# sacs-epfl/decentralized-learning-simulator

Measured on AMD Instinct MI355X. Metric: device-resident GB/s, N-way weighted model-tensor reduce; 1/2/4/8 MI355X, higher is better.
Workload: dtype f32

## Files before the change

decentralized-learning-simulator_amd/csrc/dispatch.hpp:

```cpp
#pragma once

#include <hip/hip_runtime.h>

#include <algorithm>
#include <cmath>
#include <cstdint>
#include <cstdlib>
#include <cstring>
#include <type_traits>
#include <vector>

#include "dlsim.h"
#include "wreduce_kernels.hpp"
#include "chunk_mean_kernels.hpp"
#include "ab_env.hpp"


namespace dlsim_host __attribute__((visibility("hidden"))) {

int fail(int code, const char* fmt, ...) __attribute__((format(printf, 2, 3)));
int hip_fail(hipError_t e, const char* what);

constexpr int kVpt = 4;
constexpr size_t kBatchSmallBytes = size_t{1} << 20;
// ... 446 lines not shown
    fi.push_back(fan_in[t]);
    dv.push_back(divs ? divs[t] : 1.0f);
  }
  const int g = static_cast<int>(group.size());
  const size_t tile1 = dlsim::kBlock;
  int t0 = 0;
  while (t0 < g) {
    int t1 = t0, ptrs = 0;
    uint64_t blocks = 0;
    while (t1 < g && t1 - t0 < dlsim::kBatchMaxTasks && ptrs + fi[t1] <= dlsim::kBatchMaxPtrs &&
           blocks + ne[t1] / Op::E / tile1 + 1 < 0x7fffffffull) {
      ptrs += fi[t1];
      blocks += ne[t1] / Op::E / tile1 + 1;
      ++t1;
    }
    hipError_t e = launch_batch<Op>(fi.data(), ioff.data(), ins.data(), ws.data(), dv.data(), os.data(),
                                    ne.data(), t0, t1, st);
    if (e != hipSuccess) return hip_fail(e, "batched kernel launch");
    t0 = t1;
  }
  return DLSIM_OK;
}

struct TableLayout {
  size_t tasks_off, map_off, ptrs_off, w_off, bytes;
  uint32_t nblocks;
  int vpt;
};

inline size_t round8(size_t x) { return (x + 7) / 8 * 8; }

template <class Op>
uint32_t task_blocks(size_t nelem, int vpt) {
  const size_t tile = static_cast<size_t>(dlsim::kBlock) * vpt;
  return static_cast<uint32_t>(nelem / Op::E / tile + 1);
}

template <class Op>
bool table_layout(int b, const int* fan_in, const size_t* nelem, TableLayout* L) {
  uint64_t blocks = 0, ptrs = 0;
  L->vpt = batch_vpt<Op>(nelem, 0, b);
  for (int t = 0; t < b; ++t) {
    blocks += task_blocks<Op>(nelem[t], L->vpt);
    ptrs += static_cast<uint64_t>(fan_in[t]);
  }
  if (blocks >= 0x7fffffffull) return false;
  L->nblocks = static_cast<uint32_t>(blocks);
  L->tasks_off = round8(sizeof(dlsim::BatchTableHeader));
  L->map_off = round8(L->tasks_off + sizeof(dlsim::BatchTaskDesc) * static_cast<size_t>(b));
  L->ptrs_off = round8(L->map_off + sizeof(uint32_t) * static_cast<size_t>(blocks));
  L->w_off = round8(L->ptrs_off + sizeof(void*) * static_cast<size_t>(ptrs));
  L->bytes = round8(L->w_off + sizeof(float) * static_cast<size_t>(ptrs));
  return true;
}

template <class Op>
int table_fill(int b, const int* fan_in, const void* const* in, const float* w, void* const* outs,
               const size_t* nelem, void* h_table, size_t bytes) {
  TableLayout L;
  if (!table_layout<Op>(b, fan_in, nelem, &L)) return fail(DLSIM_E_ARG, "batch too large");
  if (bytes < L.bytes) return fail(DLSIM_E_ARG, "table buffer too small (%zu < %zu)", bytes, L.bytes);
  if (cross_task_overlap(b, fan_in, in, outs, nelem, Op::kBytes))
    return fail(DLSIM_E_ARG,
                "a task's output overlaps another task's input or output: one table launch runs all tasks "
                "concurrently (use separate calls, or dlsim_wreduce_batched, which orders them)");
  unsigned char* base = static_cast<unsigned char*>(h_table);
  std::memset(base, 0, L.bytes);
  auto* h = reinterpret_cast<dlsim::BatchTableHeader*>(base);
  auto* tasks = reinterpret_cast<dlsim::BatchTaskDesc*>(base + L.tasks_off);
  auto* map = reinterpret_cast<uint32_t*>(base + L.map_off);
  auto* ptrs = reinterpret_cast<const void**>(base + L.ptrs_off);
  auto* ws = reinterpret_cast<float*>(base + L.w_off);
  h->ntasks = static_cast<uint32_t>(b);
  h->nblocks = L.nblocks;
  h->vpt = static_cast<uint32_t>(L.vpt);
  h->tasks_off = L.tasks_off;
  h->map_off = L.map_off;
  h->ptrs_off = L.ptrs_off;
  h->w_off = L.w_off;
  uint32_t blk = static_cast<uint32_t>(b), off = 0;
  bool uniform = true;
  for (int t = 0; t < b; ++t) {
    const size_t total = nelem[t] * Op::kBytes;
    if (fan_in[t] > DLSIM_MAX_FUSED_INPUTS || total > kMaxLaunchOutBytes || !aligned16(outs[t]))
      return fail(DLSIM_E_ARG, "task %d cannot be table-batched (fan-in <= %d, 16-B aligned, < 2 GiB)", t,
                  DLSIM_MAX_FUSED_INPUTS);
    const uint32_t nb = task_blocks<Op>(nelem[t], L.vpt);
    tasks[t].out = outs[t];
    tasks[t].nvec = nelem[t] / Op::E;
    tasks[t].nelem = nelem[t];
    tasks[t].block_start = blk - 1;
    tasks[t].ptr_off = off;
    tasks[t].fan_in = static_cast<uint32_t>(fan_in[t]);
    map[t] = static_cast<uint32_t>(t);
    for (uint32_t k = 0; k + 1 < nb; ++k) map[blk + k] = static_cast<uint32_t>(t);
    for (int i = 0; i < fan_in[t]; ++i) {
      if (!aligned16(in[off + i]))
        return fail(DLSIM_E_ARG, "task %d input %d is not 16-byte aligned", t, i);
      ptrs[off + i] = in[off + i];
      ws[off + i] = w[off + i];
    }
    blk += nb - 1;
    off += static_cast<uint32_t>(fan_in[t]);
    uniform = uniform && fan_in[t] == fan_in[0];
  }
  h->uniform_fan_in = uniform ? static_cast<uint32_t>(fan_in[0]) : 0u;
  return DLSIM_OK;
}

template <class Op, int NF, int VPT>
hipError_t launch_table_nf(const void* d_table, uint32_t blocks, hipStream_t st) {
  hipLaunchKernelGGL((dlsim::k_wreduce_batch_table<Op, NF, group_size<Op>(), VPT, kNT, store_policy<Op>(),
                                                    kBatchWave<Op, VPT>>),
                     dim3(blocks), dim3(dlsim::kBlock), 0, st, static_cast<const unsigned char*>(d_table));
  return hipGetLastError();
}

template <class Op, int K, int VPT>
hipError_t launch_table_fixed(const void* d_table, int n, uint32_t blocks, hipStream_t st) {
  if constexpr (K > max_fixed_fan_in<Op>()) {
    return launch_table_nf<Op, 0, VPT>(d_table, blocks, st);
  } else {
    if (n == K) return launch_table_nf<Op, K, VPT>(d_table, blocks, st);
    return launch_table_fixed<Op, K + 1, VPT>(d_table, n, blocks, st);
  }
}

template <class Op>
int table_launch(const void* h_table, const void* d_table, hipStream_t st) {
  const auto* h = static_cast<const dlsim::BatchTableHeader*>(h_table);
  if (h->ntasks == 0) return DLSIM_OK;
  if (h->vpt != 1 && h->vpt != 4)
    return fail(DLSIM_E_ARG, "not a table written by dlsim_batch_table_fill (vectors per lane %u)", h->vpt);
  const int n = static_cast<int>(h->uniform_fan_in);
  hipError_t e;
  if (h->vpt == 1)
    e = n ? launch_table_fixed<Op, 1, 1>(d_table, n, h->nblocks, st) : launch_table_nf<Op, 0, 1>(d_table, h->nblocks, st);
  else
    e = n ? launch_table_fixed<Op, 1, 4>(d_table, n, h->nblocks, st) : launch_table_nf<Op, 0, 4>(d_table, h->nblocks, st);
  if (e != hipSuccess) return hip_fail(e, "table batch launch");
  return DLSIM_OK;
}


inline size_t chunk_mean_ilp_begin(int m, size_t n, int threads, size_t esz = 4, size_t vw = 8) {
  if (n <= 1) return 0;
  const size_t rnd = 128 / esz;
  size_t b = 0, e = n;
  if (!(static_cast<unsigned long long>(m) * n < 32768ULL || threads <= 1)) {
    const size_t tp = static_cast<size_t>(threads) < n ? static_cast<size_t>(threads) : n;
    const size_t cs = (n + tp - 1) / tp;
    for (size_t t = 0; t < tp; ++t) {
      size_t tb = t * cs;
      if (tb >= n) break;
      size_t te = tb + cs < n ? tb + cs : n;
      tb -= tb % rnd;
      if (te != n) te -= te % rnd;
      if (tb < te) {
        b = tb;
        e = te;
      }
    }
  }
// ... 278 lines not shown
      continue;
    }
    if (static_cast<int>(batch.size()) == dlsim::kCmMaxTasks || np + m > dlsim::kCmMaxPtrs ||
        tiles + tb > 0x7fffffffu) {
      int rc = flush();
      if (rc != DLSIM_OK) return rc;
    }
    batch.push_back({t, ib, flags, head});
    np += m;
    tiles += tb;
  }
  return flush();
}

}

#define DLSIM_REDUCE_ENTRIES(X, Op)                                                                      \
  X int dlsim_host::run<Op>(const void* const*, int, const float*, void*, size_t, hipStream_t, float);  \
  X int dlsim_host::run_batched<Op>(int, const int*, const void* const*, const float*, void* const*,    \
                                    const size_t*, hipStream_t, const float*);                          \
  X bool dlsim_host::table_layout<Op>(int, const int*, const size_t*, dlsim_host::TableLayout*);        \
  X int dlsim_host::table_fill<Op>(int, const int*, const void* const*, const float*, void* const*,     \
                                   const size_t*, void*, size_t);                                       \
  X int dlsim_host::table_launch<Op>(const void*, const void*, hipStream_t);
#define DLSIM_MEAN_ENTRIES(X, Op)                                                                        \
  X int dlsim_host::run<Op>(const void* const*, int, const float*, void*, size_t, hipStream_t, float);  \
  X int dlsim_host::run_batched<Op>(int, const int*, const void* const*, const float*, void* const*,    \
                                    const size_t*, hipStream_t, const float*);                          \
  X int dlsim_host::run_chunk_mean<Op>(int, const int*, const void* const*, void* const*, const size_t*, \
                                       int, hipStream_t, std::vector<dlsim_host::ChunkMeanPlan>*, int);
#define DLSIM_PROBE_ENTRIES(X, Op) \
  X int dlsim_host::run<Op>(const void* const*, int, const float*, void*, size_t, hipStream_t, float);
#define DLSIM_F64_ENTRIES(X, Op) \
  X int dlsim_host::run<Op>(const void* const*, int, const double*, void*, size_t, hipStream_t, float);
#define DLSIM_CHUNK_ENTRIES(X, Op)                                                                       \
  X int dlsim_host::run_chunk_mean<Op>(int, const int*, const void* const*, void* const*, const size_t*, \
                                       int, hipStream_t, std::vector<dlsim_host::ChunkMeanPlan>*, int);

#define DLSIM_ALL_ENTRIES(X)                  \
  DLSIM_REDUCE_ENTRIES(X, dlsim::F32Exact)    \
  DLSIM_REDUCE_ENTRIES(X, dlsim::F32Fast)     \
  DLSIM_REDUCE_ENTRIES(X, dlsim::BF16Exact)   \
  DLSIM_REDUCE_ENTRIES(X, dlsim::BF16Fast)    \
  DLSIM_REDUCE_ENTRIES(X, dlsim::F16Exact)    \
  DLSIM_REDUCE_ENTRIES(X, dlsim::F16Fast)     \
  DLSIM_MEAN_ENTRIES(X, dlsim::F32Mean)       \
  DLSIM_MEAN_ENTRIES(X, dlsim::BF16Mean)      \
// ... 7 lines not shown
```

decentralized-learning-simulator_amd/csrc/dlsim_abi.hip:

```cpp
#include <hip/hip_runtime.h>

#include <algorithm>
#include <cstdarg>
#include <cstdio>
#include <cstdint>
#include <cstdlib>
#include <cstring>
#include <mutex>
#include <string>
#include <thread>
#include <vector>

#include "abi_common.hpp"
#include "dispatch.hpp"
#include "fanin_checks.hpp"

#include "host_pack.hpp"

namespace dlsim_host __attribute__((visibility("hidden"))) {

template <class F>
int with_policy(int dtype, int mode, F&& f) {
  const bool fast = mode == DLSIM_FAST;
  if (dtype == DLSIM_F32) return fast ? f(dlsim::F32Fast{}) : f(dlsim::F32Exact{});
// ... 393 lines not shown
                           size_t table_bytes) {
  g_err.clear();
  if (b < 0 || !h_table) return fail(DLSIM_E_ARG, "bad arguments");
  if (b > 0 && (!fan_in || !d_inputs || !h_weights || !d_outs || !n_elems))
    return fail(DLSIM_E_ARG, "null array argument");
  size_t off = 0;
  for (int t = 0; t < b; ++t) {
    int rc = check_args(d_inputs + off, fan_in[t], h_weights + off, d_outs[t], n_elems[t], dtype, DLSIM_EXACT);
    if (rc != DLSIM_OK) return fail(rc, "task %d: %s", t, g_err.c_str());
    off += static_cast<size_t>(fan_in[t]);
  }
  return with_policy(dtype, DLSIM_EXACT, [&](auto op) {
    return table_fill<decltype(op)>(b, fan_in, d_inputs, h_weights, d_outs, n_elems, h_table, table_bytes);
  });
}

int dlsim_batch_table_launch(const void* h_table, const void* d_table, int dtype, int mode, void* stream) {
  g_err.clear();
  if (!h_table || !d_table) return fail(DLSIM_E_ARG, "null table");
  if (!known_dtype(dtype)) return dtype_fail(dtype);
  if (mode != DLSIM_EXACT && mode != DLSIM_FAST) return fail(DLSIM_E_MODE, "unsupported mode %d", mode);
  hipStream_t st = static_cast<hipStream_t>(stream);
  return with_policy(dtype, mode, [&](auto op) { return table_launch<decltype(op)>(h_table, d_table, st); });
}

int dlsim_mean(const void* const* d_inputs, int n, void* d_out, size_t n_elems, int dtype,
               void* stream) {
  g_err.clear();
  int rc = check_args(d_inputs, n, nullptr, d_out, n_elems, dtype, DLSIM_EXACT, false);
  if (rc != DLSIM_OK) return rc;
  hipStream_t st = static_cast<hipStream_t>(stream);
  const float div = static_cast<float>(n);
  return with_mean_policy(dtype, [&](auto op) {
    return run<decltype(op)>(d_inputs, n, nullptr, d_out, n_elems, st, div);
  });
}

int dlsim_mean_batched(int b, const int* fan_in, const void* const* d_inputs, void* const* d_outs,
                       const size_t* n_elems, int dtype, void* stream) {
  g_err.clear();
  if (b < 0) return fail(DLSIM_E_ARG, "b must be >= 0 (got %d)", b);
  if (b == 0) return DLSIM_OK;
  if (!fan_in || !d_inputs || !d_outs || !n_elems) return fail(DLSIM_E_ARG, "null array argument");
  size_t off = 0;
  std::vector<float> divs(static_cast<size_t>(b));
  for (int t = 0; t < b; ++t) {
// ... 1054 lines not shown
```

decentralized-learning-simulator_amd/csrc/wreduce_kernels.hpp:

```cpp
#pragma once

#include <hip/hip_runtime.h>
#include <stdint.h>

#include <type_traits>

#pragma clang fp contract(off)

namespace dlsim {

constexpr int kBlock = 256;

typedef uint32_t u32x4 __attribute__((ext_vector_type(4)));
typedef float f32x2 __attribute__((ext_vector_type(2)));
typedef __bf16 bf16x2 __attribute__((ext_vector_type(2)));

__device__ __forceinline__ float bf16_round(float f) {
  uint32_t u = __float_as_uint(f);
  if ((u & 0x7fffffffu) > 0x7f800000u) return __uint_as_float(0x7fc00000u);
  u += 0x7fffu + ((u >> 16) & 1u);
  return __uint_as_float(u & 0xffff0000u);
}

__device__ __forceinline__ void bf16_round2(float& a0, float& a1) {
// ... 754 lines not shown
    if (full * kTile < nvec)
      reduce_tile<Op, TaskArgs, NF, G, VPT, NT, true, STP>(a, n, o, full * kTile + threadIdx.x, nvec);
    const size_t j = nvec * Op::E + threadIdx.x;
    if (j < s.nelem[t]) fold_scalar<Op, TaskArgs>(a, n, s.out[t], j);
    return;
  }
  if constexpr (WAVEMAP) {
    const size_t lane_off = (threadIdx.x >> 6) * 64 * VPT + (threadIdx.x & 63);
    reduce_tile<Op, TaskArgs, NF, G, VPT, NT, false, STP, 64>(a, n, o, (local - 1) * kTile + lane_off, nvec);
  } else {
    reduce_tile<Op, TaskArgs, NF, G, VPT, NT, false, STP>(a, n, o, (local - 1) * kTile + threadIdx.x, nvec);
  }
}

struct BatchTableHeader {
  uint32_t ntasks;
  uint32_t nblocks;
  uint32_t uniform_fan_in;
  uint32_t vpt;
  uint64_t tasks_off;
  uint64_t map_off;
  uint64_t ptrs_off;
  uint64_t w_off;
};

struct BatchTaskDesc {
  void* out;
  uint64_t nvec;
  uint64_t nelem;
  uint32_t block_start;
  uint32_t ptr_off;
  uint32_t fan_in;
  uint32_t reserved;
};

struct TableArgs {
  const void* const* p;
  const float* w;
  __device__ const void* ptr(int i) const { return p[i]; }
  __device__ float wt(int i) const { return w[i]; }
  __device__ float divisor() const { return 1.0f; }
};

template <class Op, int NF, int G, int VPT, int NT, int STP, bool WAVEMAP = false>
__global__ __launch_bounds__(kBlock) void k_wreduce_batch_table(const unsigned char* __restrict__ table) {
  const BatchTableHeader* h = reinterpret_cast<const BatchTableHeader*>(table);
  const uint32_t* map = reinterpret_cast<const uint32_t*>(table + h->map_off);
// ... 2 lines not shown
  const TableArgs a{reinterpret_cast<const void* const*>(table + h->ptrs_off) + d.ptr_off,
                    reinterpret_cast<const float*>(table + h->w_off) + d.ptr_off};
  const int n = NF > 0 ? NF : static_cast<int>(d.fan_in);
  const size_t nvec = d.nvec;
  constexpr size_t kTile = static_cast<size_t>(kBlock) * VPT;
  const size_t full = nvec / kTile;
  const OutRef o = make_out<STP>(d.out, nvec);
  const uint32_t local = blockIdx.x < h->ntasks ? 0u : blockIdx.x - d.block_start;
  if (local == 0) {
    if (full * kTile < nvec)
      reduce_tile<Op, TableArgs, NF, G, VPT, NT, true, STP>(a, n, o, full * kTile + threadIdx.x, nvec);
    const size_t j = nvec * Op::E + threadIdx.x;
    if (j < d.nelem) fold_scalar<Op, TableArgs>(a, n, d.out, j);
    return;
  }
  if constexpr (WAVEMAP) {
    const size_t lane_off = (threadIdx.x >> 6) * 64 * VPT + (threadIdx.x & 63);
    reduce_tile<Op, TableArgs, NF, G, VPT, NT, false, STP, 64>(a, n, o, (local - 1) * kTile + lane_off, nvec);
  } else {
    reduce_tile<Op, TableArgs, NF, G, VPT, NT, false, STP>(a, n, o, (local - 1) * kTile + threadIdx.x, nvec);
  }
}

template <int BYTES>
struct XorProbe {
  static constexpr int E = 16 / BYTES;
  static constexpr int kBytes = BYTES;
  static constexpr int kFmt = BYTES == 4 ? kFmtF32 : kFmtBF16;
  __device__ static float init(float) { return 0.0f; }
  __device__ static float step(float acc, float, float x) {
    float r = __uint_as_float(__float_as_uint(acc) ^ __float_as_uint(x));
    asm volatile("" : "+v"(r));
    return r;
  }
  __device__ static void step2(float& a0, float& a1, float w, float x0, float x1) {
    a0 = step(a0, w, x0);
    a1 = step(a1, w, x1);
  }
  __device__ static float finish(float a, float) { return a; }
};

constexpr int kMixedMaxInputs = 32;
struct MixedSlots {
  const void* p[kMixedMaxInputs];
  double w[kMixedMaxInputs];
  int dt[kMixedMaxInputs];
// ... 68 lines not shown
```

decentralized-learning-simulator_amd/dasklearn_amd/_native.py:

```python
from __future__ import annotations

import ctypes
import os
import threading
from typing import Optional, Sequence

import numpy as np

LIB_DIR = os.path.join(os.path.dirname(os.path.abspath(__file__)), "lib")
LIB_PATH = os.path.join(LIB_DIR, "libdlsim_hip.so")

DLSIM_F32 = 0
DLSIM_BF16 = 1
DLSIM_F16 = 2
DLSIM_F64 = 3
DLSIM_EXACT = 0
DLSIM_FAST = 1
MAX_FUSED_INPUTS = 128
DLSIM_E_ARG = -1
DLSIM_E_RCCL = -4
DLSIM_E_PEER = -5
DLSIM_E_DISAGREE = -6
DLSIM_GATHER_NONE = 0
DLSIM_GATHER_BCAST = 1
DLSIM_GATHER_ALLGATHER = 2


def ab_env(name: str, default: Optional[str] = None) -> Optional[str]:
    if os.environ.get("DLSIM_AB") != "1":
        return default
    return os.environ.get(name, default)

EXPORTS = (
    "dlsim_wreduce",
    "dlsim_wreduce_f64",
    "dlsim_wreduce_tensors",
    "dlsim_wreduce_batched",
    "dlsim_batch_table_bytes",
    "dlsim_batch_table_fill",
    "dlsim_batch_table_launch",
    "dlsim_mean",
    "dlsim_mean_batched",
    "dlsim_chunk_mean_batched",
    "dlsim_chunk_mean_ilp_begin",
    "dlsim_chunk_mean_plan",
    "dlsim_rccl_bind",
    "dlsim_wreduce_sharded",
    "dlsim_wreduce_sharded_f64",
    "dlsim_wreduce_mixed",
    "dlsim_sgd_step",
    "dlsim_sgd_step_tensors",
    "dlsim_sgd_momentum_step",
    "dlsim_sgd_momentum_step_tensors",
    "dlsim_robust_reduce",
    "dlsim_robust_reduce_tensors",
    "dlsim_robust_reduce_batched",
    "dlsim_robust_batch_geometry",
    "dlsim_robust_reduce_tensors_batched",
    "dlsim_robust_nearest_reduce",
    "dlsim_robust_nearest_reduce_tensors",
    "dlsim_pairwise_sqdist",
    "dlsim_pairwise_sqdist_tensors",
    "dlsim_pairdist_geometry",
# ... 14 lines not shown
    "dlsim_sharded_plan_run_f64",
    "dlsim_sharded_plan_destroy",
    "dlsim_host_wreduce",
    "dlsim_host_wreduce_zc",
    "dlsim_host_wreduce_resident",
    "dlsim_host_chunk_mean",
    "dlsim_host_pack",
    "dlsim_shard_range",
    "dlsim_probe_pattern",
    "dlsim_kernel_name",
    "dlsim_last_error",
    "dlsim_version",
)

_lib = None
_lock = threading.Lock()


class ChunkLaunch(ctypes.Structure):
    _fields_ = [("form", ctypes.c_int), ("mf", ctypes.c_int), ("rows", ctypes.c_int), ("bpt", ctypes.c_int),
                ("grid", ctypes.c_uint), ("ntasks", ctypes.c_int), ("first_task", ctypes.c_int)]


CHUNK_FORMS = ("tiled_few", "tiled", "table", "defer_rf4", "defer_rf8", "defer_m")


class DlsimError(RuntimeError):

    def __init__(self, fn: str, rc: int, msg: str):
        super().__init__(f"{fn} failed (rc={rc}): {msg}")
        self.rc = rc


def load() -> ctypes.CDLL:
    global _lib
    if _lib is not None:
        return _lib
    with _lock:
        if _lib is not None:
            return _lib
        if not os.path.exists(LIB_PATH):
            raise ImportError(
                f"HIP extension not built: {LIB_PATH} is missing. Run "
                "`python -c 'import __graft_entry__ as g; g.build()'` at the repo root.")
        lib = ctypes.CDLL(LIB_PATH)
        vp, sz, i = ctypes.c_void_p, ctypes.c_size_t, ctypes.c_int
        lib.dlsim_wreduce.argtypes = [ctypes.POINTER(vp), i, ctypes.POINTER(ctypes.c_float), vp,
                                      sz, i, i, vp]
        lib.dlsim_wreduce.restype = i
        lib.dlsim_wreduce_f64.argtypes = [ctypes.POINTER(vp), i, ctypes.POINTER(ctypes.c_double), vp, sz, i, vp]
        lib.dlsim_wreduce_f64.restype = i
        lib.dlsim_wreduce_tensors.argtypes = [ctypes.POINTER(vp), i, i, ctypes.POINTER(sz),
                                              ctypes.POINTER(ctypes.c_float), ctypes.POINTER(vp),
                                              i, i, vp]
        lib.dlsim_wreduce_tensors.restype = i
        lib.dlsim_wreduce_batched.argtypes = [i, ctypes.POINTER(i), ctypes.POINTER(vp),
                                              ctypes.POINTER(ctypes.c_float), ctypes.POINTER(vp),
                                              ctypes.POINTER(sz), i, i, vp]
        lib.dlsim_wreduce_batched.restype = i
        lib.dlsim_batch_table_bytes.argtypes = [i, ctypes.POINTER(i), ctypes.POINTER(sz), i,
                                                ctypes.POINTER(sz)]
        lib.dlsim_batch_table_bytes.restype = i
        lib.dlsim_batch_table_fill.argtypes = [i, ctypes.POINTER(i), ctypes.POINTER(vp),
                                               ctypes.POINTER(ctypes.c_float), ctypes.POINTER(vp),
                                               ctypes.POINTER(sz), i, vp, sz]
        lib.dlsim_batch_table_fill.restype = i
        lib.dlsim_batch_table_launch.argtypes = [vp, vp, i, i, vp]
        lib.dlsim_batch_table_launch.restype = i
        lib.dlsim_mean.argtypes = [ctypes.POINTER(vp), i, vp, sz, i, vp]
        lib.dlsim_mean.restype = i
        lib.dlsim_mean_batched.argtypes = [i, ctypes.POINTER(i), ctypes.POINTER(vp), ctypes.POINTER(vp),
                                           ctypes.POINTER(sz), i, vp]
        lib.dlsim_mean_batched.restype = i
        lib.dlsim_chunk_mean_batched.argtypes = [i, ctypes.POINTER(i), ctypes.POINTER(vp), ctypes.POINTER(vp),
                                                 ctypes.POINTER(sz), i, i, vp]
        lib.dlsim_chunk_mean_batched.restype = i
        lib.dlsim_chunk_mean_ilp_begin.argtypes = [i, sz, i]
        lib.dlsim_chunk_mean_ilp_begin.restype = sz
        lib.dlsim_chunk_mean_plan.argtypes = [i, ctypes.POINTER(i), ctypes.POINTER(vp), ctypes.POINTER(vp),
                                              ctypes.POINTER(sz), i, i, i, ctypes.POINTER(ChunkLaunch), i,
                                              ctypes.POINTER(i)]
        lib.dlsim_chunk_mean_plan.restype = i
        lib.dlsim_rccl_bind.argtypes = [ctypes.c_char_p]
        lib.dlsim_rccl_bind.restype = i
        lib.dlsim_wreduce_sharded.argtypes = [ctypes.POINTER(vp), sz, i, ctypes.POINTER(ctypes.c_float), vp, sz, i,
                                              i, vp, i, vp]
        lib.dlsim_wreduce_sharded.restype = i
        lib.dlsim_wreduce_sharded_f64.argtypes = [ctypes.POINTER(vp), sz, i, ctypes.POINTER(ctypes.c_double), vp,
                                                  sz, i, vp, i, vp]
        lib.dlsim_wreduce_sharded_f64.restype = i
        lib.dlsim_sharded_plan_create.argtypes = [vp, sz, i, i, i, vp, ctypes.POINTER(vp)]
# ... 688 lines not shown
            numels.append(out.numel())
        lib = load()
        c_fan = (ctypes.c_int * self.b)(*fan)
        c_num = (ctypes.c_size_t * self.b)(*numels)
        nbytes = ctypes.c_size_t(0)
        _check("dlsim_batch_table_bytes",
               lib.dlsim_batch_table_bytes(self.b, c_fan, c_num, self.dtype, ctypes.byref(nbytes)))
        self._h = torch.empty(nbytes.value, dtype=torch.uint8, pin_memory=True)
        _check("dlsim_batch_table_fill",
               lib.dlsim_batch_table_fill(self.b, c_fan, (ctypes.c_void_p * len(ptrs))(*ptrs),
                                          (ctypes.c_float * len(ws))(*ws),
                                          (ctypes.c_void_p * self.b)(*outs), c_num, self.dtype,
                                          self._h.data_ptr(), nbytes.value))
        self._d = self._h.to(self.device, non_blocking=True)
        torch.cuda.current_stream(self.device).synchronize()
        self._keep = tasks
        self._lib = lib

    def launch(self, stream=None) -> None:
        _check("dlsim_batch_table_launch",
               self._lib.dlsim_batch_table_launch(self._h.data_ptr(), self._d.data_ptr(), self.dtype,
                                                  self.mode, _stream_handle(self.device, stream)))


def wreduce_batched(tasks, mode: int = DLSIM_EXACT, stream=None):
    lib = load()
    b = len(tasks)
    if b == 0:
        return []
    dt = dtype_code(tasks[0][2].dtype)
    fan, ptrs, ws, outs, numels = [], [], [], [], []
    for inputs, w32, out in tasks:
        if len(inputs) < 1:
            raise IndexError("list index out of range")
        if len(w32) != len(inputs):
            raise AssertionError("weights/models length mismatch")
        for t in list(inputs) + [out]:
            if not t.is_cuda or t.dtype != out.dtype or t.numel() != out.numel() or not t.is_contiguous() \
                    or t.device != out.device:
                raise ValueError("each task: contiguous device tensors of one dtype, size and device")
        if out.dtype != tasks[0][2].dtype or out.device != tasks[0][2].device:
            raise ValueError("all tasks of a batch share dtype and device")
        fan.append(len(inputs))
        ptrs.extend(t.data_ptr() for t in inputs)
        ws.extend(np.asarray(w32, dtype=np.float32).tolist())
        outs.append(out.data_ptr())
# ... 549 lines not shown
```

include/dlsim.h:

```cpp
#ifndef DLSIM_H_
#define DLSIM_H_

#include <stddef.h>
#include <stdint.h>

#ifdef __cplusplus
extern "C" {
#endif

enum dlsim_dtype {
  DLSIM_F32 = 0,
  DLSIM_BF16 = 1,
  DLSIM_F16 = 2,
  DLSIM_F64 = 3
};

enum dlsim_mode {
  DLSIM_EXACT = 0,
  DLSIM_FAST = 1
};

#define DLSIM_OK 0
#define DLSIM_E_ARG (-1)
#define DLSIM_E_DTYPE (-2)
// ... 14 lines not shown
int dlsim_wreduce(const void* const* d_inputs, int n, const float* h_weights,
                  void* d_out, size_t n_elems, int dtype, int mode,
                  void* stream);

int dlsim_wreduce_f64(const void* const* d_inputs, int n, const double* h_weights, void* d_out, size_t n_elems,
                      int mode, void* stream);

int dlsim_wreduce_tensors(const void* const* d_inputs, int n, int t,
                          const size_t* numels, const float* h_weights,
                          void* const* d_outs, int dtype, int mode,
                          void* stream);

int dlsim_wreduce_batched(int b, const int* fan_in, const void* const* d_inputs,
                          const float* h_weights, void* const* d_outs, const size_t* n_elems,
                          int dtype, int mode, void* stream);

int dlsim_batch_table_bytes(int b, const int* fan_in, const size_t* n_elems, int dtype,
                            size_t* bytes);
int dlsim_batch_table_fill(int b, const int* fan_in, const void* const* d_inputs,
                           const float* h_weights, void* const* d_outs, const size_t* n_elems,
                           int dtype, void* h_table, size_t table_bytes);
int dlsim_batch_table_launch(const void* h_table, const void* d_table, int dtype, int mode,
                             void* stream);

int dlsim_mean(const void* const* d_inputs, int n, void* d_out, size_t n_elems, int dtype,
               void* stream);

int dlsim_mean_batched(int b, const int* fan_in, const void* const* d_inputs, void* const* d_outs,
                       const size_t* n_elems, int dtype, void* stream);

int dlsim_chunk_mean_batched(int b, const int* fan_in, const void* const* d_inputs, void* const* d_outs,
                             const size_t* n_elems, int dtype, int cpu_threads, void* stream);

size_t dlsim_chunk_mean_ilp_begin(int m, size_t n_elems, int cpu_threads);

enum {
  DLSIM_CHUNK_TILED_FEW = 0,
  DLSIM_CHUNK_TILED = 1,
  DLSIM_CHUNK_TABLE = 2,
  DLSIM_CHUNK_DEFER_RF4 = 3,
  DLSIM_CHUNK_DEFER_RF8 = 4,
  DLSIM_CHUNK_DEFER_M = 5
};
typedef struct dlsim_chunk_launch {
  int form;
  int mf;
// ... 152 lines not shown
```

Before: 6738.

## Add deferred multi-row kernel path for f32 table-batched weighted reduce

For f32 exact table batches with uniform fan-in between 3 and 10, the table fill now builds per-block records. Each record carries that block's input pointers and weights and covers R rows of a large task. A new deferred kernel reads these records into scalar registers and processes R rows per block, with R chosen so the block count fits the CU count. Small tasks fall back to the existing tiled table kernel in a second launch. The aim is fewer blocks, less per-block table lookup and better streaming, at the cost of a larger table, an extra launch for mixed batches and a changed table header format.

```diff
diff --git a/decentralized-learning-simulator_amd/csrc/dispatch.hpp b/decentralized-learning-simulator_amd/csrc/dispatch.hpp
--- a/decentralized-learning-simulator_amd/csrc/dispatch.hpp
+++ b/decentralized-learning-simulator_amd/csrc/dispatch.hpp
@@ -492,13 +492,102 @@
   return DLSIM_OK;
 }
 
-struct TableLayout {
-  size_t tasks_off, map_off, ptrs_off, w_off, bytes;
+constexpr size_t kBatchDeferMinRows = 256;
+constexpr int kBatchDeferLdsKB = 0;
+inline bool batch_defer_on() {
+  const char* e = dlsim::ab_getenv("DLSIM_BATCH_DEFER");
+  return !(e && e[0] == '0');
+}
+inline size_t batch_defer_min_rows() {
+  const char* e = dlsim::ab_getenv("DLSIM_BATCH_DEFER_MIN_ROWS");
+  return e ? static_cast<size_t>(std::max(1L, std::atol(e))) : kBatchDeferMinRows;
+}
+inline size_t batch_defer_lds_bytes() {
+  const char* e = dlsim::ab_getenv("DLSIM_BATCH_DEFER_LDS_KB");
+  const long kb = e ? std::atol(e) : kBatchDeferLdsKB;
+  return static_cast<size_t>(std::min(160L, std::max(0L, kb))) * 1024;
+}
+
+hipError_t launch_batch_defer(int nf, int R, const void* d_table, uint32_t blocks, size_t lds_bytes, hipStream_t st);
+
+struct BatchDeferPlan {
+  int nf = 0, R = 0;
+  uint32_t blocks = 0, partial = 0;
+  std::vector<int> tasks, rest;
+};
+
+template <class Op>
+bool task_has_partial(size_t nelem, int R) {
+  const size_t nvec = nelem / Op::E, rows = nvec / dlsim::kDeferBlock;
+  return rows % static_cast<size_t>(R) != 0 || nvec % dlsim::kDeferBlock != 0 || nelem % Op::E != 0;
+}
+
+template <class Op>
+BatchDeferPlan batch_defer_plan(int b, const int* fan_in, const size_t* nelem, size_t cus) {
+  BatchDeferPlan P;
+  if constexpr (!std::is_same<Op, dlsim::F32Exact>::value) {
+    return P;
+  } else {
+    if (b < 1 || cus < 1) return P;
+    const int nf = fan_in[0];
+    if (nf < dlsim::kBatchDeferMinFanIn || nf > dlsim::kBatchDeferMaxFanIn) return P;
+    for (int t = 1; t < b; ++t)
+      if (fan_in[t] != nf) return P;
+    const size_t min_rows = batch_defer_min_rows();
+    size_t rows = 0;
+    for (int t = 0; t < b; ++t) {
+      const size_t r = nelem[t] / Op::E / dlsim::kDeferBlock;
+      if (r >= min_rows && nelem[t] * Op::kBytes <= kMaxLaunchOutBytes) {
+        P.tasks.push_back(t);
+        rows += r;
+      } else {
+        P.rest.push_back(t);
+      }
+    }
+    if (rows < static_cast<size_t>(kDeferRMin) * cus) return BatchDeferPlan{};
+    auto count = [&](int R, uint64_t* partial) {
+      uint64_t nb = 0, np = 0;
+      for (int t : P.tasks) {
+        nb += nelem[t] / Op::E / dlsim::kDeferBlock / static_cast<size_t>(R);
+        np += task_has_partial<Op>(nelem[t], R) ? 1 : 0;
+      }
+      *partial = np;
+      return nb + np;
+    };
+    uint64_t np = 0;
+    int R = 0;
+    if (defer_r_override() > 0) {
+      R = std::min(std::max(defer_r_override() & ~1, kDeferRMin), dlsim::kBatchDeferRMax);
+    } else {
+      for (int r = kDeferRMin; r <= dlsim::kBatchDeferRMax && !R; r += kDeferU)
+        if (count(r, &np) <= cus) R = r;
+      if (!R) R = std::min(defer_rows(rows * dlsim::kDeferBlock, cus, dlsim::kBatchDeferRMax), dlsim::kBatchDeferRMax);
+    }
+    const uint64_t blocks = count(R, &np);
+    if (blocks >= 0x7fffffffull) return BatchDeferPlan{};
+    P.nf = nf;
+    P.R = R;
+    P.blocks = static_cast<uint32_t>(blocks);
+    P.partial = static_cast<uint32_t>(np);
+    return P;
+  }
+}
+
+struct TiledLayout {
+  size_t tasks_off, map_off, ptrs_off, w_off, end;
   uint32_t nblocks;
   int vpt;
 };
+struct TableLayout {
+  TiledLayout all;
+  BatchDeferPlan defer;
+  size_t rest_off = 0;
+  TiledLayout rest{};
+  size_t bytes = 0;
+};
 
 inline size_t round8(size_t x) { return (x + 7) / 8 * 8; }
+inline size_t round64(size_t x) { return (x + 63) / 64 * 64; }
 
 template <class Op>
 uint32_t task_blocks(size_t nelem, int vpt) {
@@ -507,7 +596,7 @@
 }
 
 template <class Op>
-bool table_layout(int b, const int* fan_in, const size_t* nelem, TableLayout* L) {
+bool tiled_layout(int b, const int* fan_in, const size_t* nelem, size_t first, TiledLayout* L) {
   uint64_t blocks = 0, ptrs = 0;
   L->vpt = batch_vpt<Op>(nelem, 0, b);
   for (int t = 0; t < b; ++t) {
@@ -516,26 +605,43 @@
   }
   if (blocks >= 0x7fffffffull) return false;
   L->nblocks = static_cast<uint32_t>(blocks);
-  L->tasks_off = round8(sizeof(dlsim::BatchTableHeader));
+  L->tasks_off = round8(first);
   L->map_off = round8(L->tasks_off + sizeof(dlsim::BatchTaskDesc) * static_cast<size_t>(b));
   L->ptrs_off = round8(L->map_off + sizeof(uint32_t) * static_cast<size_t>(blocks));
   L->w_off = round8(L->ptrs_off + sizeof(void*) * static_cast<size_t>(ptrs));
-  L->bytes = round8(L->w_off + sizeof(float) * static_cast<size_t>(ptrs));
+  L->end = round8(L->w_off + sizeof(float) * static_cast<size_t>(ptrs));
   return true;
 }
 
-template <class Op>
-int table_fill(int b, const int* fan_in, const void* const* in, const float* w, void* const* outs,
-               const size_t* nelem, void* h_table, size_t bytes) {
-  TableLayout L;
-  if (!table_layout<Op>(b, fan_in, nelem, &L)) return fail(DLSIM_E_ARG, "batch too large");
-  if (bytes < L.bytes) return fail(DLSIM_E_ARG, "table buffer too small (%zu < %zu)", bytes, L.bytes);
-  if (cross_task_overlap(b, fan_in, in, outs, nelem, Op::kBytes))
-    return fail(DLSIM_E_ARG,
-                "a task's output overlaps another task's input or output: one table launch runs all tasks "
-                "concurrently (use separate calls, or dlsim_wreduce_batched, which orders them)");
-  unsigned char* base = static_cast<unsigned char*>(h_table);
-  std::memset(base, 0, L.bytes);
+static_assert(sizeof(dlsim::BatchTableHeader) <= dlsim::kBatchRecOff, "the records start behind the header");
+
+template <class Op>
+bool table_layout(int b, const int* fan_in, const size_t* nelem, TableLayout* L) {
+  L->defer = batch_defer_plan<Op>(b, fan_in, nelem, static_cast<size_t>(device_cus()));
+  const BatchDeferPlan& P = L->defer;
+  const size_t first = P.R ? dlsim::kBatchRecOff + sizeof(dlsim::BatchDeferRec) * static_cast<size_t>(P.blocks)
+                           : sizeof(dlsim::BatchTableHeader);
+  if (!tiled_layout<Op>(b, fan_in, nelem, first, &L->all)) return false;
+  L->bytes = L->all.end;
+  L->rest_off = 0;
+  if (P.R && !P.rest.empty()) {
+    std::vector<int> fi;
+    std::vector<size_t> ne;
+    for (int t : P.rest) {
+      fi.push_back(fan_in[t]);
+      ne.push_back(nelem[t]);
+    }
+    L->rest_off = round64(L->bytes);
+    if (!tiled_layout<Op>(static_cast<int>(fi.size()), fi.data(), ne.data(), sizeof(dlsim::BatchTableHeader), &L->rest))
+      return false;
+    L->bytes = L->rest_off + L->rest.end;
+  }
+  return true;
+}
+
+template <class Op>
+int fill_tiled(unsigned char* base, const TiledLayout& L, int b, const int* idx, const int* fan_in, const size_t* in_off,
+               const void* const* in, const float* w, void* const* outs, const size_t* nelem) {
   auto* h = reinterpret_cast<dlsim::BatchTableHeader*>(base);
   auto* tasks = reinterpret_cast<dlsim::BatchTaskDesc*>(base + L.tasks_off);
   auto* map = reinterpret_cast<uint32_t*>(base + L.map_off);
@@ -548,34 +654,92 @@
   h->map_off = L.map_off;
   h->ptrs_off = L.ptrs_off;
   h->w_off = L.w_off;
+  h->format = dlsim::kBatchTableFormat;
   uint32_t blk = static_cast<uint32_t>(b), off = 0;
   bool uniform = true;
-  for (int t = 0; t < b; ++t) {
+  for (int k = 0; k < b; ++k) {
+    const int t = idx ? idx[k] : k;
     const size_t total = nelem[t] * Op::kBytes;
     if (fan_in[t] > DLSIM_MAX_FUSED_INPUTS || total > kMaxLaunchOutBytes || !aligned16(outs[t]))
       return fail(DLSIM_E_ARG, "task %d cannot be table-batched (fan-in <= %d, 16-B aligned, < 2 GiB)", t,
                   DLSIM_MAX_FUSED_INPUTS);
     const uint32_t nb = task_blocks<Op>(nelem[t], L.vpt);
-    tasks[t].out = outs[t];
-    tasks[t].nvec = nelem[t] / Op::E;
-    tasks[t].nelem = nelem[t];
-    tasks[t].block_start = blk - 1;
-    tasks[t].ptr_off = off;
-    tasks[t].fan_in = static_cast<uint32_t>(fan_in[t]);
-    map[t] = static_cast<uint32_t>(t);
-    for (uint32_t k = 0; k + 1 < nb; ++k) map[blk + k] = static_cast<uint32_t>(t);
+    tasks[k].out = outs[t];
+    tasks[k].nvec = nelem[t] / Op::E;
+    tasks[k].nelem = nelem[t];
+    tasks[k].block_start = blk - 1;
+    tasks[k].ptr_off = off;
+    tasks[k].fan_in = static_cast<uint32_t>(fan_in[t]);
+    map[k] = static_cast<uint32_t>(k);
+    for (uint32_t j = 0; j + 1 < nb; ++j) map[blk + j] = static_cast<uint32_t>(k);
     for (int i = 0; i < fan_in[t]; ++i) {
-      if (!aligned16(in[off + i]))
+      if (!aligned16(in[in_off[t] + i]))
         return fail(DLSIM_E_ARG, "task %d input %d is not 16-byte aligned", t, i);
-      ptrs[off + i] = in[off + i];
-      ws[off + i] = w[off + i];
+      ptrs[off + i] = in[in_off[t] + i];
+      ws[off + i] = w[in_off[t] + i];
     }
     blk += nb - 1;
     off += static_cast<uint32_t>(fan_in[t]);
-    uniform = uniform && fan_in[t] == fan_in[0];
-  }
-  h->uniform_fan_in = uniform ? static_cast<uint32_t>(fan_in[0]) : 0u;
+    uniform = uniform && fan_in[t] == fan_in[idx ? idx[0] : 0];
+  }
+  h->uniform_fan_in = uniform ? static_cast<uint32_t>(fan_in[idx ? idx[0] : 0]) : 0u;
   return DLSIM_OK;
+}
+
+template <class Op>
+int table_fill(int b, const int* fan_in, const void* const* in, const float* w, void* const* outs,
+               const size_t* nelem, void* h_table, size_t bytes) {
+  TableLayout L;
+  if (!table_layout<Op>(b, fan_in, nelem, &L)) return fail(DLSIM_E_ARG, "batch too large");
+  if (bytes < L.bytes) return fail(DLSIM_E_ARG, "table buffer too small (%zu < %zu)", bytes, L.bytes);
+  if (cross_task_overlap(b, fan_in, in, outs, nelem, Op::kBytes))
+    return fail(DLSIM_E_ARG,
+                "a task's output overlaps another task's input or output: one table launch runs all tasks "
+                "concurrently (use separate calls, or dlsim_wreduce_batched, which orders them)");
+  unsigned char* base = static_cast<unsigned char*>(h_table);
+  std::memset(base, 0, L.bytes);
+  std::vector<size_t> in_off(static_cast<size_t>(b) + 1, 0);
+  for (int t = 0; t < b; ++t) in_off[t + 1] = in_off[t] + static_cast<size_t>(fan_in[t]);
+  int rc = fill_tiled<Op>(base, L.all, b, nullptr, fan_in, in_off.data(), in, w, outs, nelem);
+  if (rc != DLSIM_OK) return rc;
+  const BatchDeferPlan& P = L.defer;
+  if (!P.R) return DLSIM_OK;
+  auto* h = reinterpret_cast<dlsim::BatchTableHeader*>(base);
+  h->defer_r = static_cast<uint32_t>(P.R);
+  h->defer_blocks = P.blocks;
+  h->defer_tasks = static_cast<uint32_t>(P.tasks.size());
+  h->rec_off = dlsim::kBatchRecOff;
+  auto* recs = reinterpret_cast<dlsim::BatchDeferRec*>(base + dlsim::kBatchRecOff);
+  uint32_t at_partial = 0, at_full = P.partial;
+  const size_t span = static_cast<size_t>(P.R) * dlsim::kDeferBlock;
+  for (int t : P.tasks) {
+    const size_t nvec = nelem[t] / Op::E, rows = nvec / dlsim::kDeferBlock, full = rows / static_cast<size_t>(P.R);
+    dlsim::BatchDeferRec r{};
+    r.out = outs[t];
+    r.nvec = nvec;
+    r.nelem = nelem[t];
+    for (int i = 0; i < P.nf; ++i) {
+      r.p[i] = in[in_off[t] + i];
+      r.w[i] = w[in_off[t] + i];
+    }
+    if (task_has_partial<Op>(nelem[t], P.R)) {
+      r.first = full * span;
+      r.rows = static_cast<uint32_t>(rows - full * static_cast<size_t>(P.R));
+      r.kind = dlsim::kBatchRecPartial;
+      recs[at_partial++] = r;
+    }
+    r.rows = static_cast<uint32_t>(P.R);
+    r.kind = dlsim::kBatchRecFull;
+    for (size_t k = 0; k < full; ++k) {
+      r.first = k * span;
+      recs[at_full++] = r;
+    }
+  }
+  if (at_partial != P.partial || at_full != P.blocks) return fail(DLSIM_E_ARG, "internal: deferred block count");
+  if (P.rest.empty()) return DLSIM_OK;
+  h->rest_off = L.rest_off;
+  return fill_tiled<Op>(base + L.rest_off, L.rest, static_cast<int>(P.rest.size()), P.rest.data(), fan_in,
+                        in_off.data(), in, w, outs, nelem);
 }
 
 template <class Op, int NF, int VPT>
@@ -596,12 +760,24 @@
   }
 }
 
-template <class Op>
-int table_launch(const void* h_table, const void* d_table, hipStream_t st) {
-  const auto* h = static_cast<const dlsim::BatchTableHeader*>(h_table);
+inline bool table_header_ok(const dlsim::BatchTableHeader* h) {
+  if (h->format != dlsim::kBatchTableFormat || (h->vpt != 1 && h->vpt != 4)) return false;
+  if (h->defer_r == 0) return h->rec_off == 0 && h->defer_blocks == 0 && h->rest_off == 0;
+  return h->rec_off == dlsim::kBatchRecOff && h->defer_r >= static_cast<uint32_t>(kDeferRMin) &&
+         h->defer_r <= static_cast<uint32_t>(dlsim::kBatchDeferRMax) && h->defer_r % 2 == 0 && h->defer_blocks > 0 &&
+         h->defer_blocks < 0x7fffffffu && h->uniform_fan_in >= static_cast<uint32_t>(dlsim::kBatchDeferMinFanIn) &&
+         h->uniform_fan_in <= static_cast<uint32_t>(dlsim::kBatchDeferMaxFanIn) && h->rest_off % 64 == 0 &&
+         h->tasks_off >= dlsim::kBatchRecOff + sizeof(dlsim::BatchDeferRec) * static_cast<size_t>(h->defer_blocks);
+}
+
+template <class Op>
+bool table_defers(const dlsim::BatchTableHeader* h) {
+  return std::is_same<Op, dlsim::F32Exact>::value && h->defer_r > 0 && batch_defer_on();
+}
+
+template <class Op>
+int launch_tiled_table(const dlsim::BatchTableHeader* h, const void* d_table, hipStream_t st) {
   if (h->ntasks == 0) return DLSIM_OK;
-  if (h->vpt != 1 && h->vpt != 4)
-    return fail(DLSIM_E_ARG, "not a table written by dlsim_batch_table_fill (vectors per lane %u)", h->vpt);
   const int n = static_cast<int>(h->uniform_fan_in);
   hipError_t e;
   if (h->vpt == 1)
@@ -609,6 +785,64 @@
   else
     e = n ? launch_table_fixed<Op, 1, 4>(d_table, n, h->nblocks, st) : launch_table_nf<Op, 0, 4>(d_table, h->nblocks, st);
   if (e != hipSuccess) return hip_fail(e, "table batch launch");
+  return DLSIM_OK;
+}
+
+template <class Op>
+int table_launch(const void* h_table, const void* d_table, hipStream_t st) {
+  const auto* h = static_cast<const dlsim::BatchTableHeader*>(h_table);
+  if (h->ntasks == 0) return DLSIM_OK;
+  if (!table_header_ok(h))
+    return fail(DLSIM_E_ARG, "not a table written by dlsim_batch_table_fill (format %#x, vectors per lane %u)",
+                h->format, h->vpt);
+  if (!table_defers<Op>(h)) return launch_tiled_table<Op>(h, d_table, st);
+  if (h->rest_off) {
+    const auto* hr = reinterpret_cast<const dlsim::BatchTableHeader*>(static_cast<const unsigned char*>(h_table) + h->rest_off);
+    if (!table_header_ok(hr) || hr->defer_r != 0)
+      return fail(DLSIM_E_ARG, "not a table written by dlsim_batch_table_fill (the tiled part of a mixed launch)");
+    const int rc = launch_tiled_table<Op>(hr, static_cast<const unsigned char*>(d_table) + h->rest_off, st);
+    if (rc != DLSIM_OK) return rc;
+  }
+  const hipError_t e = launch_batch_defer(static_cast<int>(h->uniform_fan_in), static_cast<int>(h->defer_r), d_table,
+                                          h->defer_blocks, batch_defer_lds_bytes(), st);
+  if (e != hipSuccess) return hip_fail(e, "deferred table batch launch");
+  return DLSIM_OK;
+}
+
+struct TablePlanInfo {
+  bool defers;
+  int R, fan_in;
+  uint32_t defer_blocks, defer_partial, defer_tasks, tiled_blocks, tiled_tasks;
+  int tiled_vpt;
+};
+template <class Op>
+int table_plan(const void* h_table, TablePlanInfo* q) {
+  const auto* h = static_cast<const dlsim::BatchTableHeader*>(h_table);
+  *q = TablePlanInfo{};
+  if (h->ntasks == 0) return DLSIM_OK;
+  if (!table_header_ok(h))
+    return fail(DLSIM_E_ARG, "not a table written by dlsim_batch_table_fill (format %#x, vectors per lane %u)",
+                h->format, h->vpt);
+  q->fan_in = static_cast<int>(h->uniform_fan_in);
+  const dlsim::BatchTableHeader* tiled = h;
+  if (table_defers<Op>(h)) {
+    q->defers = true;
+    q->R = static_cast<int>(h->defer_r);
+    q->defer_blocks = h->defer_blocks;
+    q->defer_tasks = h->defer_tasks;
+    const auto* recs = reinterpret_cast<const dlsim::BatchDeferRec*>(static_cast<const unsigned char*>(h_table) + h->rec_off);
+    for (uint32_t k = 0; k < h->defer_blocks && recs[k].kind == dlsim::kBatchRecPartial; ++k) ++q->defer_partial;
+    tiled = h->rest_off
+                ? reinterpret_cast<const dlsim::BatchTableHeader*>(static_cast<const unsigned char*>(h_table) + h->rest_off)
+                : nullptr;
+    if (tiled && (!table_header_ok(tiled) || tiled->defer_r != 0))
+      return fail(DLSIM_E_ARG, "not a table written by dlsim_batch_table_fill (the tiled part of a mixed launch)");
+  }
+  if (tiled) {
+    q->tiled_blocks = tiled->nblocks;
+    q->tiled_tasks = tiled->ntasks;
+    q->tiled_vpt = static_cast<int>(tiled->vpt);
+  }
   return DLSIM_OK;
 }
 
@@ -933,7 +1167,8 @@
   X bool dlsim_host::table_layout<Op>(int, const int*, const size_t*, dlsim_host::TableLayout*);        \
   X int dlsim_host::table_fill<Op>(int, const int*, const void* const*, const float*, void* const*,     \
                                    const size_t*, void*, size_t);                                       \
-  X int dlsim_host::table_launch<Op>(const void*, const void*, hipStream_t);
+  X int dlsim_host::table_launch<Op>(const void*, const void*, hipStream_t);                            \
+  X int dlsim_host::table_plan<Op>(const void*, dlsim_host::TablePlanInfo*);
 #define DLSIM_MEAN_ENTRIES(X, Op)                                                                        \
   X int dlsim_host::run<Op>(const void* const*, int, const float*, void*, size_t, hipStream_t, float);  \
   X int dlsim_host::run_batched<Op>(int, const int*, const void* const*, const float*, void* const*,    \
diff --git a/decentralized-learning-simulator_amd/csrc/dlsim_abi.hip b/decentralized-learning-simulator_amd/csrc/dlsim_abi.hip
--- a/decentralized-learning-simulator_amd/csrc/dlsim_abi.hip
+++ b/decentralized-learning-simulator_amd/csrc/dlsim_abi.hip
@@ -439,6 +439,29 @@
   if (mode != DLSIM_EXACT && mode != DLSIM_FAST) return fail(DLSIM_E_MODE, "unsupported mode %d", mode);
   hipStream_t st = static_cast<hipStream_t>(stream);
   return with_policy(dtype, mode, [&](auto op) { return table_launch<decltype(op)>(h_table, d_table, st); });
+}
+
+int dlsim_batch_table_plan(const void* h_table, int dtype, int mode, dlsim_table_launch* records, int max_records,
+                           int* n_records) {
+  g_err.clear();
+  if (!h_table || !n_records || max_records < 0 || (max_records > 0 && !records))
+    return fail(DLSIM_E_ARG, "bad arguments");
+  if (!known_dtype(dtype)) return dtype_fail(dtype);
+  if (mode != DLSIM_EXACT && mode != DLSIM_FAST) return fail(DLSIM_E_MODE, "unsupported mode %d", mode);
+  TablePlanInfo q;
+  const int rc = with_policy(dtype, mode, [&](auto op) { return table_plan<decltype(op)>(h_table, &q); });
+  if (rc != DLSIM_OK) return rc;
+  dlsim_table_launch out[2];
+  int n = 0;
+  if (q.tiled_blocks > 0)
+    out[n++] = dlsim_table_launch{"dlsim::k_wreduce_batch_table", 0, q.fan_in, q.tiled_vpt, q.tiled_blocks, 0u,
+                                  static_cast<int>(q.tiled_tasks)};
+  if (q.defers)
+    out[n++] = dlsim_table_launch{"dlsim::k_wreduce_batch_defer", q.R, q.fan_in, 0, q.defer_blocks, q.defer_partial,
+                                  static_cast<int>(q.defer_tasks)};
+  for (int k = 0; k < n && k < max_records; ++k) records[k] = out[k];
+  *n_records = n;
+  return DLSIM_OK;
 }
 
 int dlsim_mean(const void* const* d_inputs, int n, void* d_out, size_t n_elems, int dtype,
diff --git a/decentralized-learning-simulator_amd/csrc/inst_batch_defer.hip b/decentralized-learning-simulator_amd/csrc/inst_batch_defer.hip
--- /dev/null
+++ b/decentralized-learning-simulator_amd/csrc/inst_batch_defer.hip
@@ -0,0 +1,45 @@
+#include "dispatch.hpp"
+
+namespace dlsim_host {
+
+namespace {
+
+template <int NF, int RC>
+hipError_t launch_bd(const void* d_table, uint32_t blocks, size_t lds, hipStream_t st) {
+  auto* k = dlsim::k_wreduce_batch_defer<dlsim::F32Exact, NF, group_size<dlsim::F32Exact>(), RC, kDeferU, kStore>;
+  if (lds > 48 * 1024) {
+    const hipError_t e = hipFuncSetAttribute(reinterpret_cast<const void*>(k),
+                                             hipFuncAttributeMaxDynamicSharedMemorySize, static_cast<int>(lds));
+    if (e != hipSuccess) return e;
+  }
+  hipLaunchKernelGGL(k, dim3(blocks), dim3(dlsim::kDeferBlock), lds, st, static_cast<const unsigned char*>(d_table));
+  return hipGetLastError();
+}
+
+template <int NF, int RC>
+hipError_t pick_rc(int R, const void* d_table, uint32_t blocks, size_t lds, hipStream_t st) {
+  if constexpr (RC > dlsim::kBatchDeferRMax) {
+    return hipErrorInvalidValue;
+  } else {
+    if (R == RC) return launch_bd<NF, RC>(d_table, blocks, lds, st);
+    return pick_rc<NF, RC + kDeferU>(R, d_table, blocks, lds, st);
+  }
+}
+
+template <int NF>
+hipError_t pick_nf(int nf, int R, const void* d_table, uint32_t blocks, size_t lds, hipStream_t st) {
+  if constexpr (NF > dlsim::kBatchDeferMaxFanIn) {
+    return hipErrorInvalidValue;
+  } else {
+    if (nf == NF) return pick_rc<NF, kDeferRMin>(R, d_table, blocks, lds, st);
+    return pick_nf<NF + 1>(nf, R, d_table, blocks, lds, st);
+  }
+}
+
+}
+
+hipError_t launch_batch_defer(int nf, int R, const void* d_table, uint32_t blocks, size_t lds_bytes, hipStream_t st) {
+  return pick_nf<dlsim::kBatchDeferMinFanIn>(nf, R, d_table, blocks, lds_bytes, st);
+}
+
+}
diff --git a/decentralized-learning-simulator_amd/csrc/wreduce_kernels.hpp b/decentralized-learning-simulator_amd/csrc/wreduce_kernels.hpp
--- a/decentralized-learning-simulator_amd/csrc/wreduce_kernels.hpp
+++ b/decentralized-learning-simulator_amd/csrc/wreduce_kernels.hpp
@@ -800,7 +800,14 @@
   uint64_t map_off;
   uint64_t ptrs_off;
   uint64_t w_off;
-};
+  uint32_t format;
+  uint32_t defer_r;
+  uint32_t defer_blocks;
+  uint32_t defer_tasks;
+  uint64_t rec_off;
+  uint64_t rest_off;
+};
+constexpr uint32_t kBatchTableFormat = 0x32544244u;
 
 struct BatchTaskDesc {
   void* out;
@@ -849,6 +856,71 @@
   }
 }
 
+constexpr int kBatchDeferMinFanIn = 3, kBatchDeferMaxFanIn = 10, kBatchDeferRMax = 24;
+constexpr uint32_t kBatchRecFull = 0, kBatchRecPartial = 1;
+struct alignas(64) BatchDeferRec {
+  void* out;
+  uint64_t nvec;
+  uint64_t nelem;
+  uint64_t first;
+  uint32_t rows;
+  uint32_t kind;
+  const void* p[kBatchDeferMaxFanIn];
+  float w[kBatchDeferMaxFanIn];
+};
+static_assert(sizeof(BatchDeferRec) == 192, "three 64-byte lines per record");
+constexpr size_t kBatchRecOff = 128;
+
+using global_cptr = const __attribute__((address_space(1))) void*;
+template <int NF>
+struct RecRegs {
+  global_cptr p[NF];
+  float w[NF];
+  __device__ const void* ptr(int i) const { return (const void*)p[i]; }
+  __device__ float wt(int i) const { return w[i]; }
+  __device__ float divisor() const { return 1.0f; }
+};
+struct RecArgs {
+  const BatchDeferRec& r;
+  __device__ const void* ptr(int i) const { return r.p[i]; }
+  __device__ float wt(int i) const { return r.w[i]; }
+  __device__ float divisor() const { return 1.0f; }
+};
+
+template <class Op, int NF, int G, int RC, int U, int STP>
+__global__ __launch_bounds__(kDeferBlock) void k_wreduce_batch_defer(const unsigned char* __restrict__ table) {
+  static_assert(NF >= kBatchDeferMinFanIn && NF <= kBatchDeferMaxFanIn && RC <= kBatchDeferRMax, "record slots, bursts");
+  const BatchDeferRec& rec =
+      *reinterpret_cast<const BatchDeferRec*>(table + kBatchRecOff + static_cast<size_t>(blockIdx.x) * sizeof(BatchDeferRec));
+  RecRegs<NF> a;
+#pragma unroll
+  for (int i = 0; i < NF; ++i) {
+    a.p[i] = (global_cptr)rec.p[i];
+    a.w[i] = rec.w[i];
+  }
+  void* out = rec.out;
+  size_t nvec = rec.nvec, first = rec.first;
+  uint32_t kind = rec.kind;
+#pragma unroll
+  for (int i = 0; i < NF; ++i) asm volatile("" : "+s"(a.p[i]), "+s"(a.w[i]));
+  asm volatile("" : "+s"(out), "+s"(nvec), "+s"(first), "+s"(kind));
+  const OutRef o = make_out<STP>(out, nvec);
+  const size_t base = first + threadIdx.x;
+  if (kind == kBatchRecFull) {
+    defer_rows_c<Op, RecRegs<NF>, NF, G, RC, U, STP>(a, NF, o, base);
+    return;
+  }
+  constexpr int H = (RC / 2 + 1) & ~1;
+  const int R = static_cast<int>(rec.rows);
+  const int R1 = R < H ? R : H;
+  if (R1 > 0) defer_rows<Op, RecRegs<NF>, NF, G, H, U, STP>(a, NF, o, base, R1, nvec);
+  if (R > H) defer_rows<Op, RecRegs<NF>, NF, G, H, U, STP>(a, NF, o, base + static_cast<size_t>(H) * kDeferBlock, R - H, nvec);
+  const size_t rag = first + static_cast<size_t>(R) * kDeferBlock;
+  if (rag < nvec) reduce_tile<Op, RecRegs<NF>, NF, G, 1, 1, true, STP, kDeferBlock>(a, NF, o, rag + threadIdx.x, nvec);
+  const size_t j = nvec * Op::E + threadIdx.x;
+  if (j < rec.nelem) fold_scalar<Op, RecArgs>(RecArgs{rec}, NF, out, j);
+}
+
 template <int BYTES>
 struct XorProbe {
   static constexpr int E = 16 / BYTES;
diff --git a/decentralized-learning-simulator_amd/dasklearn_amd/_native.py b/decentralized-learning-simulator_amd/dasklearn_amd/_native.py
--- a/decentralized-learning-simulator_amd/dasklearn_amd/_native.py
+++ b/decentralized-learning-simulator_amd/dasklearn_amd/_native.py
@@ -39,6 +39,7 @@
     "dlsim_batch_table_bytes",
     "dlsim_batch_table_fill",
     "dlsim_batch_table_launch",
+    "dlsim_batch_table_plan",
     "dlsim_mean",
     "dlsim_mean_batched",
     "dlsim_chunk_mean_batched",
@@ -99,6 +100,11 @@
                 ("grid", ctypes.c_uint), ("ntasks", ctypes.c_int), ("first_task", ctypes.c_int)]
 
 
+class TableLaunch(ctypes.Structure):
+    _fields_ = [("kernel", ctypes.c_char_p), ("rows", ctypes.c_int), ("fan_in", ctypes.c_int), ("vpt", ctypes.c_int),
+                ("grid", ctypes.c_uint), ("partial_blocks", ctypes.c_uint), ("ntasks", ctypes.c_int)]
+
+
 CHUNK_FORMS = ("tiled_few", "tiled", "table", "defer_rf4", "defer_rf8", "defer_m")
 
 
@@ -144,6 +150,8 @@
         lib.dlsim_batch_table_fill.restype = i
         lib.dlsim_batch_table_launch.argtypes = [vp, vp, i, i, vp]
         lib.dlsim_batch_table_launch.restype = i
+        lib.dlsim_batch_table_plan.argtypes = [vp, i, i, ctypes.POINTER(TableLaunch), i, ctypes.POINTER(i)]
+        lib.dlsim_batch_table_plan.restype = i
         lib.dlsim_mean.argtypes = [ctypes.POINTER(vp), i, vp, sz, i, vp]
         lib.dlsim_mean.restype = i
         lib.dlsim_mean_batched.argtypes = [i, ctypes.POINTER(i), ctypes.POINTER(vp), ctypes.POINTER(vp),
@@ -878,6 +886,18 @@
                self._lib.dlsim_batch_table_launch(self._h.data_ptr(), self._d.data_ptr(), self.dtype,
                                                   self.mode, _stream_handle(self.device, stream)))
 
+    def launches(self):
+        return table_launches(self._h.data_ptr(), self.dtype, self.mode)
+
+
+def table_launches(h_table_ptr: int, dtype: int, mode: int = DLSIM_EXACT):
+    lib = load()
+    recs = (TableLaunch * 2)()
+    n = ctypes.c_int(0)
+    _check("dlsim_batch_table_plan", lib.dlsim_batch_table_plan(h_table_ptr, dtype, mode, recs, 2, ctypes.byref(n)))
+    return [{"kernel": r.kernel.decode(), "rows": r.rows, "fan_in": r.fan_in, "vpt": r.vpt, "grid": r.grid,
+             "partial_blocks": r.partial_blocks, "ntasks": r.ntasks} for r in recs[:n.value]]
+
 
 def wreduce_batched(tasks, mode: int = DLSIM_EXACT, stream=None):
     lib = load()
diff --git a/include/dlsim.h b/include/dlsim.h
--- a/include/dlsim.h
+++ b/include/dlsim.h
@@ -60,6 +60,18 @@
                            int dtype, void* h_table, size_t table_bytes);
 int dlsim_batch_table_launch(const void* h_table, const void* d_table, int dtype, int mode,
                              void* stream);
+
+typedef struct dlsim_table_launch {
+  const char* kernel;
+  int rows;
+  int fan_in;
+  int vpt;
+  unsigned grid;
+  unsigned partial_blocks;
+  int ntasks;
+} dlsim_table_launch;
+int dlsim_batch_table_plan(const void* h_table, int dtype, int mode, dlsim_table_launch* records,
+                           int max_records, int* n_records);
 
 int dlsim_mean(const void* const* d_inputs, int n, void* d_out, size_t n_elems, int dtype,
                void* stream);
```

Measured after the change: 6736. About the same (-0.0%).
